# MaxHalford/sorobn

Hardware: NVIDIA H100
Metric: exact-inference queries/sec (higher is better)
Workload: dtype f32

## Files before the change

sorobn_b200/csrc/sbn_api.cu:

```cuda
#include <cuda_runtime.h>

#include <algorithm>
#include <cmath>
#include <cstdarg>
#include <cstdio>
#include <cstdlib>
#include <cstring>
#include <string>
#include <vector>

#include "sbn_chain.h"
#include "sbn_count.cuh"
#include "sbn_deriv.cuh"
#include "sbn_gibbs.cuh"
#include "sbn_internal.h"
#include "sbn_join.h"
#include "sbn_kernels.cuh"
#include "sbn_launch.h"
#include "sbn_marginal.cuh"
#include "sbn_mpe.cuh"
#include "sbn_pair.h"
#include "sbn_sample.cuh"
#include "sbn_soft.cuh"
#include "sbn_tma.h"
// ... 1095 lines not shown
        sbn_soft_pack<float><<<grid, threads, 0, stream>>>(static_cast<const float *>(P->lik), P->ld_lik, rows, n_soft,
                                                           P->d_soft, P->d_arena, P->ld, P->d_log_max);
    return cudaGetLastError();
}

inline bool hoisted(const sbn_program *P, const StepDesc &st) { return P->mode == 1 && st.kind == 0; }

inline bool chain_on(const sbn_program *P) {
    return P->use_chain && P->chain_fits && P->use_tiled && !P->use_branches && !P->segments.empty();
}

inline bool pair_on(const sbn_program *P) {
    return P->use_pair && P->use_tiled && !P->use_branches && (!chain_on(P) || P->pairs_avoid_segments) && !P->pairs.empty();
}

int run_table_steps(sbn_program *P) {
    if (P->mode != 1) return SBN_OK;
    SbnStep q;
    for (const StepDesc &st : P->steps) {
        if (!hoisted(P, st)) continue;
        build_params(P, st, nullptr, 0, 1, &q);
        SBN_CUDA(launch_step(P, st, q, P->stream));
    }
    SBN_CUDA(cudaStreamSynchronize(P->stream));
    P->setup_launches = P->launches;
    P->launches = 0;
    return SBN_OK;
}

inline bool fold_normalise(const sbn_program *P, const StepDesc &st, const SbnStep &q) {
#if !SBN_FOLD_NORMALISE
    (void)P;
    (void)st;
    (void)q;
    return false;
#endif
    static const bool enabled = [] {
        const char *e = getenv("SOROBN_B200_FOLD_NORMALISE");
        return e ? atoi(e) != 0 : true;
    }();
    return enabled && P->kind == kPosterior && !P->f64 && P->post_batched && st.kind == 1 && q.tile_off != nullptr &&
           q.slab_off == nullptr && st.n_tiles == 1 && st.n_out == P->Q && !sbn_tma_eligible(P, st);
}

int issue_all(sbn_program *P, const uint8_t *d_ev, int64_t ld_ev, int64_t n_rows, float *d_out, int64_t ld_out,
              cudaStream_t stream, cudaEvent_t *events, const DrawnCodes &dc = {}) {
    if (P->kind == kSample) SBN_CUDA(cudaMemsetAsync(dc.flags(P), 0, static_cast<size_t>(n_rows), stream));
    if (!P->soft.empty()) SBN_CUDA(launch_soft_pack(P, n_rows, stream));
    SbnStep q;
    int k = 0;
    int n_decoded = 0;
    bool folded = false;
    bool skip_second = false;
    for (const StepDesc &st : P->steps) {
        if (events) SBN_CUDA(cudaEventRecord(events[k], stream));
        ++k;
        if (hoisted(P, st)) continue;
        if (P->forward_run && !P->forward[k - 1]) continue;
        if (st.kind >= 2) {
            const int decoded = st.kind == 4 || st.kind == 5 ? n_decoded++ : 0;
            SBN_CUDA(launch_kind_step(P, st, decoded, d_ev, ld_ev, n_rows, d_out, ld_out, dc, stream));
            continue;
        }
        const int seg = chain_on(P) ? P->seg_first[k - 1] : -1;
        if (seg == -2) continue;
        if (seg >= 0) {
            P->launches++;
            SBN_CUDA(sbn_chain_launch(P, *P->segments[seg], d_ev, ld_ev, n_rows, d_out, ld_out, stream));
            continue;
        }
        int pair = pair_on(P) ? P->pair_first[k - 1] : -1;
        if (pair == -2 && !skip_second) pair = -1;
        skip_second = false;
        if (pair == -2) continue;
        if (pair >= 0 && !sbn_pair_fits(P, *P->pairs[pair])) pair = -1;
        if (pair >= 0) {
            skip_second = true;
            P->launches++;
            SBN_CUDA(sbn_pair_launch(P, *P->pairs[pair], d_ev, ld_ev, n_rows, stream));
            continue;
        }
        build_params(P, st, d_ev, ld_ev, n_rows, &q);
        if (k == static_cast<int>(P->steps.size()) && fold_normalise(P, st, q)) {
            q.norm_out = d_out;
            q.norm_ld = ld_out;
            q.norm_totals = P->d_total;
            q.norm_min = SBN_MIN_TOTAL_F32;
            folded = true;
        }
        SBN_CUDA(launch_step(P, st, q, stream));
    }
    if (events) SBN_CUDA(cudaEventRecord(events[k], stream));
    switch (P->kind) {
        case kPosterior:
            if (!folded && !(chain_on(P) && P->segments.back()->ends_in_posterior))
                SBN_CUDA(launch_normalise(P, d_out, ld_out, n_rows, stream));
            break;
        case kCounts:
        case kGrad: SBN_CUDA(launch_prob(P, n_rows, d_out, nullptr, stream)); break;
        case kSample: SBN_CUDA(launch_prob(P, n_rows, d_out, dc.flags(P), stream)); break;
        case kMarginals:
        case kMpe:
        case kMap: break;
    }
    if (events) SBN_CUDA(cudaEventRecord(events[k + 1], stream));
    return SBN_OK;
}

int issue_branched(sbn_program *P, const uint8_t *d_ev, int64_t ld_ev, int64_t n_rows, float *d_out, int64_t ld_out,
                   cudaStream_t origin) {
    const int n_steps = static_cast<int>(P->steps.size());
    const int n_slots = static_cast<int>(P->slots.size());
    std::vector<int> last_writer(n_slots, -1);
    std::vector<std::vector<int>> readers(n_slots);
    std::vector<int> stream_of(n_steps, 0);
    cudaEvent_t fork = P->step_done[n_steps];
    if (!P->soft.empty()) SBN_CUDA(launch_soft_pack(P, n_rows, origin));
    SBN_CUDA(cudaEventRecord(fork, origin));
    bool joined[sbn_program::kBranches] = {false, false, false, false};
    int rr = 0;
    SbnStep q;
    for (int s = 0; s < n_steps; ++s) {
        const StepDesc &st = P->steps[s];
        if (hoisted(P, st)) continue;
        std::vector<int> deps;
        int home = -1;
        int64_t home_size = -1;
        for (const InDesc &in : st.in) {
// ... 227 lines not shown
    if (n_table_floats > 0) {
        SBN_CUDA_P(cudaMalloc(&P->d_tables, static_cast<size_t>(n_table_floats) * elem));
        SBN_CUDA_P(cudaMemcpyAsync(P->d_tables, tables, static_cast<size_t>(n_table_floats) * elem,
                                   cudaMemcpyHostToDevice, P->stream));
    }
    int64_t shared_floats = 0;
    for (Slot &s : P->slots)
        if (!s.batched) shared_floats += round_up(s.padded, 64);
    if (shared_floats > 0) {
        SBN_CUDA_P(cudaMalloc(&P->d_shared, static_cast<size_t>(shared_floats) * elem));
        SBN_CUDA_P(cudaMemsetAsync(P->d_shared, 0, static_cast<size_t>(shared_floats) * elem, P->stream));
        int64_t off = 0;
        for (Slot &s : P->slots)
            if (!s.batched) {
                s.ptr = reinterpret_cast<float *>(reinterpret_cast<char *>(P->d_shared) + off * elem);
                off += round_up(s.padded, 64);
            }
    }
    {
        std::vector<int32_t> &tile_words = P->h_tile_words;
        tile_words.clear();
        plan_tiles(P, &tile_words);
        if (!tile_words.empty()) {
            SBN_CUDA_P(cudaMalloc(&P->d_tile_off, tile_words.size() * 4));
            SBN_CUDA_P(cudaMemcpyAsync(P->d_tile_off, tile_words.data(), tile_words.size() * 4,
                                       cudaMemcpyHostToDevice, P->stream));
        }
        SBN_CUDA_P(cudaStreamSynchronize(P->stream));
        if (P->kind == kPosterior && P->soft.empty()) sbn_chain_plan(P);
    }
    if (!P->soft.empty()) {
        P->use_tma = false;
        std::vector<int32_t> desc;
        for (const auto &sv : P->soft) {
            int64_t off = 0;
            for (int s = 0; s < sv.first; ++s)
                if (P->slots[s].batched) off += P->slots[s].size;
            desc.push_back(static_cast<int32_t>(off));
            desc.push_back(sv.second);
        }
        SBN_CUDA_P(cudaMalloc(&P->d_soft, desc.size() * 4));
        SBN_CUDA_P(cudaMemcpyAsync(P->d_soft, desc.data(), desc.size() * 4, cudaMemcpyHostToDevice, P->stream));
        SBN_CUDA_P(cudaStreamSynchronize(P->stream));
    }
    {
        static bool done[64] = {false};
        if (device < 64 && !done[device]) {
            SBN_CUDA_P(sbn_batched_set_attrs());
            SBN_CUDA_P(set_tiled_attrs());
            SBN_CUDA_P(sbn_chain_set_attrs());
            SBN_CUDA_P(sbn_tma_set_attrs());
            SBN_CUDA_P(sbn_join_set_attrs());
            SBN_CUDA_P(sbn_triple_rows_set_attrs());
            SBN_CUDA_P(sbn_marginal_set_attrs());
            SBN_CUDA_P(sbn_count_set_attrs());
            SBN_CUDA_P(sbn_deriv_set_attrs());
            SBN_CUDA_P(sbn_sample_set_attrs());
            SBN_CUDA_P(sbn_argmax_set_attrs());
            SBN_CUDA_P(sbn_batched_logdomain_set_attrs());
            done[device] = true;
        }
    }
    if (P->kind == kCounts || P->kind == kGrad) {
        for (const StepDesc &st : P->steps)
            if (st.kind == 3)
                P->partial_doubles = std::max<int64_t>(P->partial_doubles, count_grid(P, st, INT32_MAX) * SBN_COUNT_WARPS * st.span);
        SBN_CUDA_P(cudaMalloc(&P->d_counts, static_cast<size_t>(P->n_counts) * 8));
    }
#undef SBN_CUDA_P
    rc = run_table_steps(P);
    if (rc != SBN_OK) return bail(rc);
    {
        cudaError_t e = P->kind == kPosterior ? sbn_pair_plan(P) : cudaSuccess;
        if (e != cudaSuccess) return bail(fail(SBN_E_CUDA, "planning the paired steps failed: %s", cudaGetErrorString(e)));
    }
    *out = P;
    return SBN_OK;
}

int sbn_program_create(int device, const int32_t *words, int64_t n_words, const float *tables, int64_t n_table_floats,
                       sbn_program **out) {
    return create_common(device, words, n_words, tables, n_table_floats, false, out);
}

int sbn_program_create_f64(int device, const int32_t *words, int64_t n_words, const double *tables,
                           int64_t n_table_doubles, sbn_program **out) {
    return create_common(device, words, n_words, tables, n_table_doubles, true, out);
}

void sbn_program_destroy(sbn_program *P) {
    if (!P) return;
    cudaSetDevice(P->device);
    free_scratch(P);
    sbn_chain_free(P);
    sbn_pair_free(P);
    cudaFree(P->d_shared);
    cudaFree(P->d_counts);
    cudaFree(P->d_partial);
    cudaFree(P->d_drawn);
    cudaFree(P->d_sample_args);
    cudaFree(P->d_soft);
    cudaFree(P->d_tile_off);
    cudaFree(P->d_tables);
    if (P->stream) cudaStreamDestroy(P->stream);
    for (auto &b : P->branch)
        if (b) cudaStreamDestroy(b);
// ... 621 lines not shown
int sbn_program_mpe_soft_host(sbn_program *P, const uint8_t *ev, int64_t ld_ev, int64_t n_rows, const double *lik,
                              int64_t ld_lik, int lik_on_device, uint8_t *codes, double *log_prob) {
    if (!log_prob) return fail(SBN_E_INVALID, "null output");
    std::vector<float> lp(n_rows > 0 ? static_cast<size_t>(n_rows) : 0);
    std::vector<double> log_max(lp.size());
    const SoftLik soft = {true, lik, ld_lik, lik_on_device, log_max.data()};
    const int rc = sample_host_common(P, ev, ld_ev, n_rows, 1, 0, 0, codes, lp.data(), false, kMpe, soft);
    if (rc != SBN_OK) return rc;
    for (size_t i = 0; i < lp.size(); ++i) log_prob[i] = static_cast<double>(lp[i]) + log_max[i];
    return SBN_OK;
}

int sbn_program_profile(sbn_program *P, const uint8_t *d_ev, int64_t ld_ev, int64_t n_rows, float *d_out,
                        int64_t ld_out, void *stream_, float *step_ms, int64_t n_step_ms) {
    int rc = check_run_args(P, d_ev, ld_ev, n_rows, d_out, ld_out);
    if (rc != SBN_OK) return rc;
    if (P->f64) return fail(SBN_E_INVALID, "profiling is for float32 programs");
    const int64_t n = static_cast<int64_t>(P->steps.size()) + 1;
    if (!step_ms || n_step_ms < n) return fail(SBN_E_INVALID, "step_ms needs %lld entries", (long long)n);
    rc = reserve_rows(P, n_rows);
    if (rc != SBN_OK) return rc;
    if (n_rows > P->reserved_rows) return fail(SBN_E_NOMEM, "n_rows exceeds the scratch that fits the device");
    cudaStream_t stream = static_cast<cudaStream_t>(stream_);
    std::vector<cudaEvent_t> ev(n + 1);
    for (auto &e : ev) SBN_CUDA(cudaEventCreate(&e));
    rc = issue_all(P, d_ev, ld_ev, n_rows, d_out, ld_out, stream, ev.data());
    if (rc == SBN_OK) {
        cudaError_t e = cudaStreamSynchronize(stream);
        if (e != cudaSuccess) rc = fail(SBN_E_CUDA, "profile run failed: %s", cudaGetErrorString(e));
    }
    if (rc == SBN_OK)
        for (int64_t i = 0; i < n; ++i) cudaEventElapsedTime(&step_ms[i], ev[i], ev[i + 1]);
    for (auto &e : ev) cudaEventDestroy(e);
    return rc;
}

int sbn_program_info(const sbn_program *P, int64_t *info, int64_t n_info) {
    if (!P || !info || n_info < 8) return fail(SBN_E_INVALID, "info needs at least 8 entries");
    if (n_info >= 12) {
        int64_t covered = 0, hbm = 0, scratch = 0;
        for (const SbnSegment *seg : P->segments) {
            covered += static_cast<int64_t>(seg->steps.size());
            hbm += seg->hbm_bytes_per_row;
            scratch = std::max(scratch, seg->scratch_floats);
        }
        info[8] = chain_on(P) ? static_cast<int64_t>(P->segments.size()) : 0;
        info[9] = chain_on(P) ? covered : 0;
        info[10] = chain_on(P) ? hbm : 0;
        info[11] = scratch;
    }
    if (n_info >= 14) {
        int64_t saved = 0;
        for (const SbnPair *pr : P->pairs) saved += 8 * P->steps[pr->step1].n_out;
        info[12] = pair_on(P) ? static_cast<int64_t>(P->pairs.size()) : 0;
        info[13] = pair_on(P) ? saved : 0;
    }
    info[0] = P->Q;
    info[1] = P->n_ev;
    info[2] = static_cast<int64_t>(P->steps.size());
    info[3] = batched_floats_per_row(P);
    info[4] = P->reserved_rows;
    info[5] = P->launches;
    info[6] = P->mode;
    int64_t shared = 0;
    for (const Slot &s : P->slots)
        if (!s.batched) shared += s.size;
    info[7] = shared;
    return SBN_OK;
}

int sbn_program_step_roles(const sbn_program *P, int32_t *roles, int64_t n_roles) {
    if (!P || !roles || n_roles < static_cast<int64_t>(P->steps.size())) return fail(SBN_E_INVALID, "roles needs n_steps entries");
    int first_kind = 0;
    bool second_follows = false;
    for (size_t i = 0; i < P->steps.size(); ++i) {
        const StepDesc &st = P->steps[i];
        if (P->mode != 1 || hoisted(P, st)) {
            roles[i] = 0;
            continue;
        }
        roles[i] = 1;
        if (chain_on(P) && P->seg_first[i] != -1) {
            roles[i] = 6;
            continue;
        }
        int pair = pair_on(P) ? P->pair_first[i] : -1;
        if (pair == -2 && !second_follows) pair = -1;
        second_follows = false;
        if (pair == -2) roles[i] = first_kind == 1 ? 5 : 3;
        if (pair >= 0 && sbn_pair_fits(P, *P->pairs[pair])) {
            first_kind = P->pairs[pair]->kind;
            roles[i] = first_kind == 1 ? 4 : 2;
            second_follows = true;
        }
    }
    return SBN_OK;
}

int sbn_program_set_graph(sbn_program *P, int enabled) {
    if (!P) return fail(SBN_E_INVALID, "null program");
    P->use_graph = enabled != 0;
    P->use_branches = enabled == 3;
    drop_graphs(P);
    return SBN_OK;
}

// ... 395 lines not shown
```

sorobn_b200/csrc/sbn_internal.h:

```cpp
#pragma once
#include <cuda_runtime.h>
#include <stdint.h>

#include <string>
#include <utility>
#include <vector>

#include "../../include/sorobn_b200.h"

struct EvAxis {
    int col, stride, card;
};
struct InDesc {
    bool is_slot;
    int id;
    bool batched;
    int sx;
    std::vector<EvAxis> ev;
    std::vector<int> estrides;
    std::vector<int> strides;
};
struct StepDesc {
    int kind;
    int out_slot;
    int cx;
    int64_t n_out;
    std::vector<int> cards;
    std::vector<int> ecards;
    int64_t zoff_pos = -1;
    int64_t zoff_tiled_pos = -1;
    std::vector<InDesc> in;
    int tile = 0;
    int nu = 0, na = 0, nb = 0, nc = 0;
    std::vector<int> order;
    int64_t n_tiles = 0;
    int64_t tile_off_pos = 0;
    bool slab = false;
    bool big_tables = false;
    int slab_ma = 0, n_slab = 0;
    int64_t slab_off_pos = 0;
    int64_t slab_tile_off_pos = 0;
    int64_t tiles_per_super = 0, n_super = 0;
    int64_t slice_pos = -1;
    int64_t slice_tpc = 0;
    int64_t slice_smem = 0;
    int64_t q_offset = -1;
    int n_common = 0;
    std::vector<EvAxis> key;
    std::vector<int> cstrides;
    int64_t span = 0;
    int64_t soff_pos = -1, coff_pos = -1;
    bool logsumexp = false;
};
struct Slot {
    bool batched;
    int64_t size;
    int64_t padded;
    float *ptr;
};

inline int64_t round_up(int64_t v, int64_t m) { return (v + m - 1) / m * m; }

struct SbnSegment;
struct SbnPair;

enum ProgramKind {
    kPosterior,
    kMarginals,
    kCounts,
    kSample,
    kMpe,
    kMap,
    kGrad,
};

inline bool sbn_log_domain(ProgramKind k) { return k == kMpe || k == kMap; }

struct GraphKey {
    const void *ev = nullptr;
    int64_t ld_ev = 0, n_rows = 0;
    const void *out = nullptr;
    int64_t ld_out = 0;
    const void *partial = nullptr;
    const void *drawn = nullptr;
    int64_t n_draws = 0, ld_drawn = 0;
    const void *lik = nullptr;
    int64_t ld_lik = 0;
    const void *weight = nullptr;
    bool operator==(const GraphKey &o) const {
        return ev == o.ev && out == o.out && ld_ev == o.ld_ev && n_rows == o.n_rows && ld_out == o.ld_out &&
               partial == o.partial && drawn == o.drawn && n_draws == o.n_draws && ld_drawn == o.ld_drawn &&
               lik == o.lik && ld_lik == o.ld_lik && weight == o.weight;
    }
};
struct CachedGraph {
    cudaGraphExec_t exec = nullptr;
    GraphKey key;
    int64_t launches = 0;
};

struct sbn_program {
    int device = 0;
    int n_sms = 1;
    bool f64 = false;
    ProgramKind kind = kPosterior;
    int mode = 0, n_ev = 0, Q = 0, post_slot = 0, post_batched = 0;
    int64_t n_counts = 0;
    int64_t n_table_floats = 0;
    double *d_counts = nullptr;
    double *d_partial = nullptr;
    int64_t partial_doubles = 0;
    int n_sampled = 0;
    uint8_t *d_drawn = nullptr;
    int64_t drawn_bytes = 0;
    uint32_t *d_sample_args = nullptr;
    std::vector<std::pair<int, int>> soft;
    int n_lik = 0;
// ... 2 lines not shown
    double *d_log_max = nullptr;
    const void *lik = nullptr;
    int64_t ld_lik = 0;
    std::vector<char> forward;
    double *d_weight = nullptr;
    const double *weight = nullptr;
    bool forward_run = false;
    CachedGraph forward_graph;
    std::vector<std::pair<int64_t, int64_t>> tables;
    std::vector<int64_t> table_padded;
    float *d_tables = nullptr;
    std::vector<Slot> slots;
    std::vector<StepDesc> steps;

    int64_t reserved_rows = 0;
    int64_t ld = 0;
    float *d_arena = nullptr;
    float *d_shared = nullptr;
    int32_t *d_tile_off = nullptr;
    float *d_total = nullptr;
    uint8_t *d_ev = nullptr;
    float *d_out = nullptr;
    cudaStream_t stream = nullptr;
    static constexpr int kBranches = 4;
    cudaStream_t branch[kBranches] = {nullptr, nullptr, nullptr, nullptr};
    std::vector<cudaEvent_t> step_done;
    std::vector<cudaEvent_t> pipe_events;
    bool use_branches = false;

    bool use_graph = true;
    bool use_tiled = true;
    bool use_slab = true;
    bool use_preload = true;
    CachedGraph graph;
    CachedGraph pipe_graph;

    int64_t launches = 0;
    int64_t setup_launches = 0;

    std::vector<SbnSegment *> segments;
    std::vector<int> seg_first;
    float *d_chain_scratch = nullptr;
    bool use_chain = true;
    bool use_tma = true;
    bool chain_fits = true;
    std::vector<int32_t> h_tile_words;

    std::vector<SbnPair *> pairs;
    std::vector<int> pair_first;
    float *d_pair_canon = nullptr;
    int32_t *d_pair_tiles = nullptr;
    bool use_pair = true;
    bool pairs_avoid_segments = false;
};
```

sorobn_b200/csrc/sbn_pair.cu:

```cuda
#include "sbn_pair.h"

#include <algorithm>
#include <cstdlib>
#include <cstring>

#include "sbn_internal.h"
#include "sbn_kernels.cuh"
#include "sbn_launch.h"

namespace {

constexpr int kV = 2;

__device__ __forceinline__ void pair_coef8(float (&c)[SBN_PAIR_PW], const float *s) {
    const float4 lo = *reinterpret_cast<const float4 *>(s);
    const float4 hi = *reinterpret_cast<const float4 *>(s + 4);
    c[0] = lo.x, c[1] = lo.y, c[2] = lo.z, c[3] = lo.w;
    c[4] = hi.x, c[5] = hi.y, c[6] = hi.z, c[7] = hi.w;
}

template <int V>
__device__ __forceinline__ void pair_ev_offsets(const SbnPairParams &p, const SbnPairEv &d, int b, int (&e)[V]) {
#pragma unroll
    for (int l = 0; l < V; ++l) e[l] = 0;
// ... 105 lines not shown
    PairG G;
    G.p = p.g + b;
    G.base = 0;
    if constexpr (M1 == SBN_PAIR_GB || M1 == SBN_PAIR_GC) {
#pragma unroll
        for (int d = 0; d < T; ++d) {
            G.x[d] = static_cast<uint32_t>(d * p.g_x) * ld;
            G.d0[d] = static_cast<uint32_t>(d * p.g_y) * ld;
            G.d1[d] = static_cast<uint32_t>(d * p.g_w) * ld;
        }
    }
    const int t_begin = chunk * p.tiles_per_cta;
    const int t_end = min(p.n_tiles, t_begin + p.tiles_per_cta);

    for (int t = t_begin; t < t_end; ++t) {
        const int4 r0 = __ldg(reinterpret_cast<const int4 *>(p.tile_off) + 2 * t);
        const int4 r1 = __ldg(reinterpret_cast<const int4 *>(p.tile_off) + 2 * t + 1);
        const uint32_t ob = static_cast<uint32_t>(r0.x) * ld, fb = static_cast<uint32_t>(r0.y) * ld;

        float f[T][T][V];
#pragma unroll
        for (int x = 0; x < T; ++x)
#pragma unroll
            for (int y = 0; y < T; ++y) sbn_ldv<V>(f[x][y], fp + (fb + xs[x] + ys[y]));
        if (p.has_pre1) {
            const float *const k = s_canon + r1.x;
#pragma unroll
            for (int x = 0; x < T; ++x)
#pragma unroll
                for (int y = 0; y < T; ++y)
#pragma unroll
                    for (int l = 0; l < V; ++l) f[x][y][l] *= k[g1[l] + x * T + y];
        }
        float mid[T][T][V];
        if constexpr (M1 == SBN_PAIR_GB || M1 == SBN_PAIR_GC) G.base = static_cast<uint32_t>(r1.z) * ld;
        pair_step<M1, V>(f, mid, s_canon + r0.z, e1, G);
        if (p.has_pre2) {
            const float *const k = s_canon + r1.y;
#pragma unroll
            for (int y = 0; y < T; ++y)
#pragma unroll
                for (int w = 0; w < T; ++w)
#pragma unroll
                    for (int l = 0; l < V; ++l) mid[y][w][l] *= k[g2[l] + y * T + w];
        }
        float acc[T][T][V];
        pair_step<M2, V>(mid, acc, s_canon + r0.w, e2, G);

#pragma unroll
        for (int z = 0; z < T; ++z)
#pragma unroll
            for (int w = 0; w < T; ++w)
                if (w < p.cw && z < p.cz) sbn_stv<V>(op + (ob + ow[w] + oz[z]), acc[w][z]);
    }
}

template <int MINB>
__global__ void __launch_bounds__(SBN_TRIPLE_THREADS, MINB) sbn_triple_kernel(const __grid_constant__ SbnTripleParams p) {
    constexpr int T = SBN_PAIR_T;
    sbn_pdl_entry();
    const int rblock = blockIdx.x / p.n_chunks;
    const int chunk = blockIdx.x % p.n_chunks;
    const int b = rblock * static_cast<int>(blockDim.x) + threadIdx.x;
    if (b >= p.n_rows) return;
    const uint32_t ld = static_cast<uint32_t>(p.ld);
    const int g = threadIdx.y;
    const float *const ap = p.a + b + static_cast<uint32_t>(g * p.a_g) * ld;
    const float *const bp = p.b + b;
    const float *const cp = p.c + b;
    float *const op = p.out + b + static_cast<uint32_t>(g * p.o_g) * ld;
    uint32_t ak[T], aj[T], bj[T], bs[T], ck[T], cz[T];
#pragma unroll
    for (int d = 0; d < T; ++d) {
        ak[d] = static_cast<uint32_t>(d * p.a_k) * ld, aj[d] = static_cast<uint32_t>(d * p.a_j) * ld;
        bj[d] = static_cast<uint32_t>(d * p.b_j) * ld, bs[d] = static_cast<uint32_t>(d * p.b_s) * ld;
        ck[d] = static_cast<uint32_t>(d * p.c_k) * ld, cz[d] = static_cast<uint32_t>(d * p.c_z) * ld;
    }
    const uint32_t oz = static_cast<uint32_t>(p.o_z) * ld, os = static_cast<uint32_t>(p.o_s) * ld;
    const int t_begin = chunk * p.tiles_per_cta;
    const int t_end = min(p.n_tiles, t_begin + p.tiles_per_cta);
    for (int t = t_begin; t < t_end; ++t) {
        const int4 row = __ldg(reinterpret_cast<const int4 *>(p.tile_off) + t);
        float acc[T][T];
#pragma unroll
        for (int z = 0; z < T; ++z)
#pragma unroll
            for (int s = 0; s < T; ++s) acc[z][s] = 0.f;
#pragma unroll 1
        for (int pp = 0; pp < T; ++pp) {
            float A[T][T], B[T][T], C[T][T];
            const uint32_t a0 = static_cast<uint32_t>(row.y + pp * p.a_p) * ld, b0 = static_cast<uint32_t>(row.z + pp * p.b_p) * ld,
                           c0 = static_cast<uint32_t>(row.w + pp * p.c_p) * ld;
#pragma unroll
            for (int j = 0; j < T; ++j)
#pragma unroll
                for (int s = 0; s < T; ++s) B[j][s] = bp[b0 + bj[j] + bs[s]];
#pragma unroll
            for (int k = 0; k < T; ++k)
#pragma unroll
                for (int j = 0; j < T; ++j) A[k][j] = ap[a0 + ak[k] + aj[j]];
#pragma unroll
            for (int k = 0; k < T; ++k)
#pragma unroll
                for (int z = 0; z < T; ++z) C[k][z] = cp[c0 + ck[k] + cz[z]];
#pragma unroll
            for (int k = 0; k < T; ++k) {
// ... 250 lines not shown
            kg = k;
    int64_t n_tiles = 1;
    std::vector<int> r2;
    for (int k = 0; k < n2; ++k)
        if (k != ks && k != kz && k != kg) r2.push_back(k), n_tiles *= s2.cards[k];
    if (n_tiles >= (1LL << 27)) return nullptr;

    SbnPair *pr = new SbnPair();
    memset(&pr->q, 0, sizeof pr->q);
    memset(&pr->t, 0, sizeof pr->t);
    pr->kind = 1;
    pr->step1 = i1, pr->step2 = i2;
    pr->g_in = -1;
    pr->a_in = ai, pr->b_in = 1 - ai, pr->c_in = 1 - mi;
    pr->tile_off_pos = static_cast<int64_t>(tiles->size());
    SbnTripleParams &q = pr->t;
    q.n_tiles = static_cast<int32_t>(n_tiles);
    q.a_j = A.estrides[0], q.a_k = A.strides[jk], q.a_p = A.strides[jp];
    q.b_j = B.estrides[0], q.b_s = B.strides[to1[ks]], q.b_p = B.strides[jp];
    q.c_k = C.estrides[kk], q.c_p = C.estrides[1 - kk], q.c_z = C.strides[kz];
    int64_t os = 1;
    std::vector<int64_t> os2(n2);
    for (int k = 0; k < n2; ++k) os2[k] = os, os *= s2.cards[k];
    q.o_z = static_cast<int32_t>(os2[kz]);
    q.o_s = static_cast<int32_t>(os2[ks]);
    q.group = kg >= 0 ? T : 1;
    q.o_g = kg >= 0 ? static_cast<int32_t>(os2[kg]) : 0;
    q.a_g = kg >= 0 ? A.strides[to1[kg]] : 0;
    std::vector<int> dig(r2.size(), 0);
    for (int64_t t = 0; t < n_tiles; ++t) {
        int64_t ob = 0, ab = 0, bb = 0, cb = 0;
        for (size_t k = 0; k < r2.size(); ++k) {
            const int ax = r2[k];
            ob += dig[k] * os2[ax];
            cb += static_cast<int64_t>(dig[k]) * C.strides[ax];
            if (to1[ax] >= 0) {
                ab += static_cast<int64_t>(dig[k]) * A.strides[to1[ax]];
                bb += static_cast<int64_t>(dig[k]) * B.strides[to1[ax]];
            }
        }
        tiles->push_back(static_cast<int32_t>(ob));
        tiles->push_back(static_cast<int32_t>(ab));
        tiles->push_back(static_cast<int32_t>(bb));
        tiles->push_back(static_cast<int32_t>(cb));
        for (size_t k = 0; k < dig.size(); ++k) {
            if (++dig[k] < s2.cards[r2[k]]) break;
            dig[k] = 0;
        }
    }
    sbn_triple_rows_plan(q, tiles->data() + pr->tile_off_pos, &pr->rows);
    return pr;
}

}

cudaError_t sbn_pair_set_attrs() {
    return cudaSuccess;
}

void sbn_pair_free(sbn_program *P) {
    for (SbnPair *pr : P->pairs) delete pr;
    P->pairs.clear();
    P->pair_first.clear();
    cudaFree(P->d_pair_canon);
    cudaFree(P->d_pair_tiles);
    P->d_pair_canon = nullptr;
    P->d_pair_tiles = nullptr;
}

cudaError_t sbn_pair_plan(sbn_program *P) {
    constexpr int T = SBN_PAIR_T;
    P->pair_first.assign(P->steps.size(), -1);
    if (P->mode != 1 || P->f64) return cudaSuccess;
    static const int min_card = [] {
        const char *e = getenv("SOROBN_B200_PAIR_MIN_CARD");
        return e ? atoi(e) : 4;
    }();

    static const bool triples_on = [] {
        const char *e = getenv("SOROBN_B200_TRIPLE");
        return e ? atoi(e) != 0 : true;
    }();

    HostTables H;
    std::vector<float> canon;
    std::vector<int32_t> tiles;
    cudaError_t err = cudaSuccess;
    bool fetched = false;

    const int n_steps = static_cast<int>(P->steps.size());
    auto launched = [&](int i) { return P->steps[i].kind != 0; };
    P->pairs_avoid_segments = P->use_chain && !P->segments.empty();
    auto in_segment = [&](int i) { return P->pairs_avoid_segments && P->seg_first[i] != -1; };
    for (int i1 = 0; i1 < n_steps; ++i1) {
        if (!launched(i1) || P->pair_first[i1] != -1) continue;
        int i2 = i1 + 1;
        while (i2 < n_steps && !launched(i2)) ++i2;
        if (i2 >= n_steps) break;
        if (in_segment(i1) || in_segment(i2)) continue;
        const StepDesc &s1 = P->steps[i1], &s2 = P->steps[i2];
        if (triples_on) {
            if (SbnPair *tr = plan_triple(P, i1, i2, &tiles)) {
                P->pair_first[i1] = static_cast<int>(P->pairs.size());
                P->pair_first[i2] = -2;
                P->pairs.push_back(tr);
                continue;
            }
        }
        if (s1.kind != 1 || s2.kind != 1 || s1.ecards.size() != 1 || s2.ecards.size() != 1) continue;
        if (s1.tile == 0 || s2.tile == 0) continue;
        int fi = -1, gi = -1, mi = -1, n_b1 = 0, n_b2 = 0;
        for (int i = 0; i < static_cast<int>(s1.in.size()); ++i)
            if (s1.in[i].batched) gi = fi, fi = i, ++n_b1;
        for (int i = 0; i < static_cast<int>(s2.in.size()); ++i)
            if (s2.in[i].batched) mi = i, ++n_b2;
        if (n_b1 < 1 || n_b1 > 2 || n_b2 != 1) continue;
// ... 70 lines not shown
            q.canon_floats = static_cast<int32_t>(total);
            const int64_t at_c1 = 0, at_c2 = c1.floats(), at_g1 = at_c2 + c2.floats(), at_g2 = at_g1 + g1.floats();
            canon.resize(canon.size() + static_cast<size_t>(total), 0.f);
            fill_canon(c1, canon.data() + pr->canon_pos + at_c1);
            fill_canon(c2, canon.data() + pr->canon_pos + at_c2);
            fill_canon(g1, canon.data() + pr->canon_pos + at_g1);
            fill_canon(g2, canon.data() + pr->canon_pos + at_g2);
            q.n_tiles = static_cast<int32_t>(n_tiles);
            q.f_sx = F.estrides[0];
            q.f_sy = F.strides[jy];
            q.cx = cx, q.cy = cy, q.cw = s2.cards[kw], q.cz = s2.cards[kz];
            int64_t os = 1;
            std::vector<int64_t> os2(n2);
            for (int k = 0; k < n2; ++k) os2[k] = os, os *= s2.cards[k];
            q.o_sw = static_cast<int32_t>(os2[kw]);
            q.o_sz = static_cast<int32_t>(os2[kz]);
            if (gi >= 0) q.g_x = s1.in[gi].estrides[0], q.g_y = s1.in[gi].strides[jy], q.g_w = s1.in[gi].strides[jw];
            q.has_pre1 = g1.tabs.empty() ? 0 : 1;
            q.has_pre2 = g2.tabs.empty() ? 0 : 1;
            set_ev(&q.ev_main1, c1);
            set_ev(&q.ev_main2, c2);
            set_ev(&q.ev_pre1, g1);
            set_ev(&q.ev_pre2, g2);
            std::vector<int> dig(r2.size(), 0);
            for (int64_t t = 0; t < n_tiles; ++t) {
                int64_t ob = 0, fb = 0;
                for (size_t k = 0; k < r2.size(); ++k) {
                    ob += dig[k] * os2[r2[k]];
                    fb += static_cast<int64_t>(dig[k]) * F.strides[r1[k]];
                }
                tiles.push_back(static_cast<int32_t>(ob));
                tiles.push_back(static_cast<int32_t>(fb));
                tiles.push_back(static_cast<int32_t>(at_c1 + tile_slab(c1, r1, dig)));
                tiles.push_back(static_cast<int32_t>(at_c2 + tile_slab(c2, r2, dig)));
                tiles.push_back(static_cast<int32_t>(at_g1 + tile_slab(g1, r1, dig)));
                tiles.push_back(static_cast<int32_t>(at_g2 + tile_slab(g2, r2, dig)));
                int64_t gb = 0;
                if (gi >= 0)
                    for (size_t k = 0; k < r1.size(); ++k) gb += static_cast<int64_t>(dig[k]) * s1.in[gi].strides[r1[k]];
                tiles.push_back(static_cast<int32_t>(gb));
                tiles.push_back(0);
                for (size_t k = 0; k < dig.size(); ++k) {
                    if (++dig[k] < s2.cards[r2[k]]) break;
                    dig[k] = 0;
                }
            }
            P->pair_first[i1] = static_cast<int>(P->pairs.size());
            P->pair_first[i2] = -2;
            P->pairs.push_back(pr);
            break;
        }
    }
    if (P->pairs.empty()) return cudaSuccess;
    err = cudaMalloc(&P->d_pair_canon, std::max<size_t>(canon.size(), 4) * 4);
    if (err != cudaSuccess) return err;
    err = cudaMalloc(&P->d_pair_tiles, tiles.size() * 4);
    if (err != cudaSuccess) return err;
    if (!canon.empty()) err = cudaMemcpy(P->d_pair_canon, canon.data(), canon.size() * 4, cudaMemcpyHostToDevice);
    if (err != cudaSuccess) return err;
    return cudaMemcpy(P->d_pair_tiles, tiles.data(), tiles.size() * 4, cudaMemcpyHostToDevice);
}

static cudaError_t triple_launch(sbn_program *P, const SbnPair &pr, int64_t n_rows, cudaStream_t stream) {
    SbnTripleParams q = pr.t;
    const StepDesc &s1 = P->steps[pr.step1], &s2 = P->steps[pr.step2];
    q.a = P->slots[s1.in[pr.a_in].id].ptr;
    q.b = P->slots[s1.in[pr.b_in].id].ptr;
    q.c = P->slots[s2.in[pr.c_in].id].ptr;
    q.out = P->slots[s2.out_slot].ptr;
    q.ld = P->ld;
    q.n_rows = static_cast<int32_t>(n_rows);
    q.tile_off = P->d_pair_tiles + pr.tile_off_pos;
    if (sbn_triple_rows_launch(P, pr.rows, q, stream)) return cudaGetLastError();
    const int rows_per_cta = q.group > 1 ? 32 : 128;
    const int64_t n_rblocks = (n_rows + rows_per_cta - 1) / rows_per_cta;
    static const int64_t tpc_env = [] {
        const char *e = getenv("SOROBN_B200_TRIPLE_TPC");
        return e ? atoll(e) : 1LL;
    }();
    static const int minb = [] {
        const char *e = getenv("SOROBN_B200_TRIPLE_MINB");
        return e ? atoi(e) : 3;
    }();
    const int64_t tpc = std::max<int64_t>(1, std::min<int64_t>(q.n_tiles, tpc_env));
    q.tiles_per_cta = static_cast<int32_t>(tpc);
    q.n_chunks = static_cast<int32_t>((q.n_tiles + tpc - 1) / tpc);
    const int64_t grid = q.n_chunks * n_rblocks;
    if (grid >= (1LL << 31)) return cudaErrorInvalidConfiguration;
    const dim3 g(static_cast<unsigned>(grid)), b(rows_per_cta, q.group);
    if (minb == 3) sbn_launch(sbn_triple_kernel<3>, g, b, 0, stream, q);
    else if (minb == 1) sbn_launch(sbn_triple_kernel<1>, g, b, 0, stream, q);
    else sbn_launch(sbn_triple_kernel<2>, g, b, 0, stream, q);
    return cudaGetLastError();
}

bool sbn_pair_fits(const sbn_program *P, const SbnPair &pr) {
    const StepDesc &s1 = P->steps[pr.step1], &s2 = P->steps[pr.step2];
    int64_t entries = P->slots[s2.out_slot].size;
    for (const InDesc &in : s1.in)
        if (in.batched) entries = std::max(entries, P->slots[in.id].size);
    for (const InDesc &in : s2.in)
        if (in.batched && in.id != s1.out_slot) entries = std::max(entries, P->slots[in.id].size);
    const char *e = getenv("SOROBN_B200_PAIR_IDX_LIMIT");
    const int64_t limit = e ? atoll(e) : (1LL << 31);
    return entries * P->ld < limit;
}

cudaError_t sbn_pair_launch(sbn_program *P, const SbnPair &pr, const uint8_t *d_ev, int64_t ld_ev, int64_t n_rows,
                            cudaStream_t stream) {
    if (pr.kind == 1) return triple_launch(P, pr, n_rows, stream);
    SbnPairParams q = pr.q;
    const StepDesc &s1 = P->steps[pr.step1], &s2 = P->steps[pr.step2];
    q.f = P->slots[s1.in[pr.f_in].id].ptr;
    q.g = pr.g_in >= 0 ? P->slots[s1.in[pr.g_in].id].ptr : q.f;
    q.out = P->slots[s2.out_slot].ptr;
    q.ev = d_ev;
    q.ld_ev = ld_ev;
    q.ld = P->ld;
    q.n_rows = static_cast<int32_t>(n_rows);
    q.canon = P->d_pair_canon + pr.canon_pos;
    q.tile_off = P->d_pair_tiles + pr.tile_off_pos;
    const int64_t n_rblocks = (n_rows + SBN_PAIR_ROWS - 1) / SBN_PAIR_ROWS;
    static const int64_t target_env = [] {
        const char *e = getenv("SOROBN_B200_PAIR_CTAS");
        return e ? atoll(e) : 0LL;
    }();
    const int64_t target = target_env > 0 ? target_env : 8LL * P->n_sms * 6;
    const int64_t chunks = std::max<int64_t>(1, std::min<int64_t>(q.n_tiles, target / std::max<int64_t>(1, n_rblocks)));
    const int64_t tpc = (q.n_tiles + chunks - 1) / chunks;
    q.tiles_per_cta = static_cast<int32_t>(tpc);
    q.n_chunks = static_cast<int32_t>((q.n_tiles + tpc - 1) / tpc);
    const int64_t grid = q.n_chunks * n_rblocks;
    if (grid >= (1LL << 31)) return cudaErrorInvalidConfiguration;
    launch_modes(pr, q, static_cast<unsigned>(grid), static_cast<size_t>(q.canon_floats) * 4, stream);
    return cudaGetLastError();
}
```

sorobn_b200/csrc/sbn_pair.h:

```cpp
#pragma once
#include <cuda_runtime.h>
#include <stdint.h>

#include <vector>

#include "../../include/sorobn_b200.h"

#define SBN_PAIR_T 5
#define SBN_PAIR_PW 8
#define SBN_PAIR_MAX_EV 4
#define SBN_PAIR_ROWS 256
#define SBN_TRIPLE_THREADS 160
#define SBN_PAIR_SMEM_MAX (40 * 1024)

struct SbnPairEv {
    int32_t n;
    int32_t col[SBN_PAIR_MAX_EV], stride[SBN_PAIR_MAX_EV], card[SBN_PAIR_MAX_EV];
};

struct SbnPairParams {
    const float *f;
    float *out;
    const uint8_t *ev;
    const float *canon;
// ... 3 lines not shown
    int32_t canon_floats;
    int32_t n_tiles, tiles_per_cta, n_chunks;
    int32_t f_sx, f_sy;
    int32_t cx, cy, cw, cz;
    int32_t o_sw, o_sz;
    int32_t has_pre1, has_pre2;
    SbnPairEv ev_main1, ev_main2, ev_pre1, ev_pre2;
    const float *g;
    int32_t g_x, g_y, g_w;
};

enum SbnPairMode { SBN_PAIR_B = 0, SBN_PAIR_CU = 1, SBN_PAIR_CE = 2, SBN_PAIR_GB = 3, SBN_PAIR_GC = 4 };

struct SbnTripleParams {
    const float *a, *b, *c;
    float *out;
    const int32_t *tile_off;
    int64_t ld;
    int32_t n_rows;
    int32_t n_tiles, tiles_per_cta, n_chunks;
    int32_t a_p, a_k, a_j;
    int32_t b_p, b_j, b_s;
    int32_t c_p, c_k, c_z;
    int32_t o_z, o_s;
    int32_t group;
    int32_t a_g, o_g;
};

#define SBN_TRIPLE_ROWS_R 16
#define SBN_TRIPLE_ROWS_COMBOS 25
#define SBN_TRIPLE_ROWS_MIN_COMBOS 8
struct SbnTripleRows {
    int ok;
    int n_combos;
    int32_t u_card[3], u_stride[3];
    int32_t u_dig[3][SBN_TRIPLE_ROWS_COMBOS];
    int32_t o_off[SBN_TRIPLE_ROWS_COMBOS];
};

struct SbnPair {
    int kind;
    int step1, step2;
    int f_in;
    int g_in;
    int m1, m2;
    SbnPairParams q;
    SbnTripleParams t;
    SbnTripleRows rows;
    int a_in, b_in, c_in;
    int64_t tile_off_pos;
    int64_t canon_pos;
};

struct sbn_program;
cudaError_t sbn_pair_plan(sbn_program *P);
cudaError_t sbn_pair_launch(sbn_program *P, const SbnPair &pr, const uint8_t *d_ev, int64_t ld_ev, int64_t n_rows,
                            cudaStream_t stream);
bool sbn_pair_fits(const sbn_program *P, const SbnPair &pr);
cudaError_t sbn_pair_set_attrs();
void sbn_pair_free(sbn_program *P);

void sbn_triple_rows_plan(const SbnTripleParams &q, const int32_t *tiles, SbnTripleRows *rows);
bool sbn_triple_rows_launch(const sbn_program *P, const SbnTripleRows &rows, const SbnTripleParams &q, cudaStream_t stream);
cudaError_t sbn_triple_rows_set_attrs();
```

Before: 25.03 million.

## Fuse consecutive pair launches into one chain kernel with shared-memory intermediates

After: 26.42 million (median of 6 runs). 1.06x the previous value.

```diff
diff --git a/sorobn_b200/csrc/sbn_api.cu b/sorobn_b200/csrc/sbn_api.cu
--- a/sorobn_b200/csrc/sbn_api.cu
+++ b/sorobn_b200/csrc/sbn_api.cu
@@ -1171,11 +1171,13 @@
     int n_decoded = 0;
     bool folded = false;
     bool skip_second = false;
+    int chain_through = -1;
     for (const StepDesc &st : P->steps) {
         if (events) SBN_CUDA(cudaEventRecord(events[k], stream));
         ++k;
         if (hoisted(P, st)) continue;
         if (P->forward_run && !P->forward[k - 1]) continue;
+        if (k - 1 <= chain_through) continue;
         if (st.kind >= 2) {
             const int decoded = st.kind == 4 || st.kind == 5 ? n_decoded++ : 0;
             SBN_CUDA(launch_kind_step(P, st, decoded, d_ev, ld_ev, n_rows, d_out, ld_out, dc, stream));
@@ -1193,6 +1195,18 @@
         skip_second = false;
         if (pair == -2) continue;
         if (pair >= 0 && !sbn_pair_fits(P, *P->pairs[pair])) pair = -1;
+        if (pair >= 0 && P->chain_at[pair] >= 0) {
+            const SbnPairChain &ch = P->pair_chains[P->chain_at[pair]];
+            bool fits = true;
+            for (int j = 1; j < ch.n; ++j) fits = fits && sbn_pair_fits(P, *P->pairs[ch.first + j]);
+            cudaError_t err = cudaSuccess;
+            if (fits && sbn_pair_chain_launch(P, ch, d_ev, ld_ev, n_rows, stream, &err)) {
+                SBN_CUDA(err);
+                P->launches++;
+                chain_through = ch.last_step;
+                continue;
+            }
+        }
         if (pair >= 0) {
             skip_second = true;
             P->launches++;
@@ -1526,6 +1540,7 @@
             SBN_CUDA_P(sbn_tma_set_attrs());
             SBN_CUDA_P(sbn_join_set_attrs());
             SBN_CUDA_P(sbn_triple_rows_set_attrs());
+            SBN_CUDA_P(sbn_pair_set_attrs());
             SBN_CUDA_P(sbn_marginal_set_attrs());
             SBN_CUDA_P(sbn_count_set_attrs());
             SBN_CUDA_P(sbn_deriv_set_attrs());
@@ -2253,6 +2268,7 @@
     if (n_info >= 14) {
         int64_t saved = 0;
         for (const SbnPair *pr : P->pairs) saved += 8 * P->steps[pr->step1].n_out;
+        for (const SbnPairChain &ch : P->pair_chains) saved += ch.saved_per_row;
         info[12] = pair_on(P) ? static_cast<int64_t>(P->pairs.size()) : 0;
         info[13] = pair_on(P) ? saved : 0;
     }
diff --git a/sorobn_b200/csrc/sbn_internal.h b/sorobn_b200/csrc/sbn_internal.h
--- a/sorobn_b200/csrc/sbn_internal.h
+++ b/sorobn_b200/csrc/sbn_internal.h
@@ -7,6 +7,7 @@
 #include <vector>
 
 #include "../../include/sorobn_b200.h"
+#include "sbn_pair.h"
 
 struct EvAxis {
     int col, stride, card;
@@ -62,7 +63,6 @@
 inline int64_t round_up(int64_t v, int64_t m) { return (v + m - 1) / m * m; }
 
 struct SbnSegment;
-struct SbnPair;
 
 enum ProgramKind {
     kPosterior,
@@ -171,4 +171,6 @@
     int32_t *d_pair_tiles = nullptr;
     bool use_pair = true;
     bool pairs_avoid_segments = false;
+    std::vector<SbnPairChain> pair_chains;
+    std::vector<int> chain_at;
 };
diff --git a/sorobn_b200/csrc/sbn_pair.cu b/sorobn_b200/csrc/sbn_pair.cu
--- a/sorobn_b200/csrc/sbn_pair.cu
+++ b/sorobn_b200/csrc/sbn_pair.cu
@@ -181,6 +181,172 @@
 #pragma unroll
             for (int w = 0; w < T; ++w)
                 if (w < p.cw && z < p.cz) sbn_stv<V>(op + (ob + ow[w] + oz[z]), acc[w][z]);
+    }
+}
+
+template <int V>
+__device__ __forceinline__ void pair_step_m(int mode, const float (&in)[SBN_PAIR_T][SBN_PAIR_T][V],
+                                            float (&acc)[SBN_PAIR_T][SBN_PAIR_T][V], const float *k, const int (&e)[V],
+                                            const PairG &G) {
+    switch (mode) {
+        case SBN_PAIR_B: pair_step<SBN_PAIR_B, V>(in, acc, k, e, G); break;
+        case SBN_PAIR_CU: pair_step<SBN_PAIR_CU, V>(in, acc, k, e, G); break;
+        case SBN_PAIR_CE: pair_step<SBN_PAIR_CE, V>(in, acc, k, e, G); break;
+        case SBN_PAIR_GB: pair_step<SBN_PAIR_GB, V>(in, acc, k, e, G); break;
+        default: pair_step<SBN_PAIR_GC, V>(in, acc, k, e, G); break;
+    }
+}
+
+struct SbnPairChainParams {
+    SbnPairParams q[SBN_PAIR_CHAIN_MAX];
+    int32_t m1[SBN_PAIR_CHAIN_MAX], m2[SBN_PAIR_CHAIN_MAX];
+    int32_t n_pairs;
+    int32_t canon_floats;
+    int32_t front_floats;
+    int32_t tiles;
+};
+
+constexpr int kChainR = SBN_PAIR_CHAIN_R;
+constexpr int kChainThreads = SBN_PAIR_CHAIN_TILES * SBN_PAIR_CHAIN_R / kV;
+
+__device__ __forceinline__ void chain_stage_canon(float *dst, const SbnPairParams &q) {
+    for (int i = threadIdx.x; i < q.canon_floats / 4; i += blockDim.x)
+        asm volatile("cp.async.cg.shared.global [%0], [%1], 16;" ::"r"(sbn_smem_u32(dst + 4 * i)), "l"(q.canon + 4 * i)
+                     : "memory");
+    asm volatile("cp.async.commit_group;" ::: "memory");
+}
+__device__ __forceinline__ void chain_canon_wait() { asm volatile("cp.async.wait_all;" ::: "memory"); }
+
+__global__ void __launch_bounds__(kChainThreads, SBN_PAIR_CHAIN_MINB) sbn_pair_chain_kernel(const __grid_constant__ SbnPairChainParams p) {
+    constexpr int T = SBN_PAIR_T, V = kV, R = kChainR, RT = R / V;
+    extern __shared__ __align__(16) float s_mem[];
+    float *const s_canon = s_mem;
+    float *const s_front = s_mem + p.canon_floats;
+    int *const s_evo = reinterpret_cast<int *>(s_front + p.front_floats);
+    int4 *const s_tiles = reinterpret_cast<int4 *>(s_evo + SBN_PAIR_CHAIN_MAX * 4 * R);
+    sbn_pdl_launch_dependents();
+
+    const int rg = threadIdx.x % RT, t = threadIdx.x / RT;
+    const int b = blockIdx.x * R + rg * V;
+    const bool live = b < p.q[0].n_rows;
+    float *const fs = s_front + rg * V;
+    chain_stage_canon(s_canon, p.q[0]);
+    for (int i = threadIdx.x; i < p.n_pairs * 4 * RT; i += blockDim.x) {
+        const int j = i / (4 * RT), a = i / RT % 4, g = i % RT;
+        const SbnPairParams &q = p.q[j];
+        const SbnPairEv &d = a == 0 ? q.ev_main1 : a == 1 ? q.ev_main2 : a == 2 ? q.ev_pre1 : q.ev_pre2;
+        const int bb = blockIdx.x * R + g * V;
+        int e[V];
+        pair_ev_offsets<V>(q, d, bb, e);
+#pragma unroll
+        for (int l = 0; l < V; ++l) s_evo[(j * 4 + a) * R + g * V + l] = e[l];
+    }
+    for (int i = threadIdx.x; i < p.n_pairs * p.tiles * 2; i += blockDim.x) {
+        const int j = i / (p.tiles * 2), k = i % (p.tiles * 2);
+        if (k < 2 * p.q[j].n_tiles) s_tiles[i] = __ldg(reinterpret_cast<const int4 *>(p.q[j].tile_off) + k);
+    }
+    chain_canon_wait();
+    __syncthreads();
+    sbn_pdl_wait();
+
+    for (int j = 0; j < p.n_pairs; ++j) {
+        const SbnPairParams &q = p.q[j];
+        const bool mine = live && t < q.n_tiles;
+        const bool last = j + 1 == p.n_pairs;
+        const uint32_t ld = static_cast<uint32_t>(q.ld);
+        float acc[T][T][V];
+        int4 r0 = make_int4(0, 0, 0, 0);
+        if (mine) {
+            int e1[V], e2[V], g1[V], g2[V];
+            const int *const ev = s_evo + j * 4 * R + rg * V;
+#pragma unroll
+            for (int l = 0; l < V; ++l) e1[l] = ev[l], e2[l] = ev[R + l], g1[l] = ev[2 * R + l], g2[l] = ev[3 * R + l];
+            r0 = s_tiles[(j * p.tiles + t) * 2];
+            const int4 r1 = s_tiles[(j * p.tiles + t) * 2 + 1];
+            float f[T][T][V];
+            if (j == 0) {
+                const float *const fp = q.f + b;
+                const uint32_t fb = static_cast<uint32_t>(r0.y) * ld;
+                uint32_t xs[T], ys[T];
+#pragma unroll
+                for (int d = 0; d < T; ++d) {
+                    xs[d] = static_cast<uint32_t>(min(d, q.cx - 1) * q.f_sx) * ld;
+                    ys[d] = static_cast<uint32_t>(min(d, q.cy - 1) * q.f_sy) * ld;
+                }
+#pragma unroll
+                for (int x = 0; x < T; ++x)
+#pragma unroll
+                    for (int y = 0; y < T; ++y) sbn_ldv<V>(f[x][y], fp + (fb + xs[x] + ys[y]));
+            } else {
+#pragma unroll
+                for (int x = 0; x < T; ++x)
+#pragma unroll
+                    for (int y = 0; y < T; ++y) {
+                        const int e = r0.y + min(x, q.cx - 1) * q.f_sx + min(y, q.cy - 1) * q.f_sy;
+                        const float2 v = *reinterpret_cast<const float2 *>(fs + e * R);
+                        f[x][y][0] = v.x, f[x][y][1] = v.y;
+                    }
+            }
+            if (q.has_pre1) {
+                const float *const k = s_canon + r1.x;
+#pragma unroll
+                for (int x = 0; x < T; ++x)
+#pragma unroll
+                    for (int y = 0; y < T; ++y)
+#pragma unroll
+                        for (int l = 0; l < V; ++l) f[x][y][l] *= k[g1[l] + x * T + y];
+            }
+            PairG G;
+            G.p = q.g + b;
+            G.base = 0;
+            if (p.m1[j] >= SBN_PAIR_GB) {
+                G.base = static_cast<uint32_t>(r1.z) * ld;
+#pragma unroll
+                for (int d = 0; d < T; ++d) {
+                    G.x[d] = static_cast<uint32_t>(d * q.g_x) * ld;
+                    G.d0[d] = static_cast<uint32_t>(d * q.g_y) * ld;
+                    G.d1[d] = static_cast<uint32_t>(d * q.g_w) * ld;
+                }
+            }
+            float mid[T][T][V];
+            pair_step_m<V>(p.m1[j], f, mid, s_canon + r0.z, e1, G);
+            if (q.has_pre2) {
+                const float *const k = s_canon + r1.y;
+#pragma unroll
+                for (int y = 0; y < T; ++y)
+#pragma unroll
+                    for (int w = 0; w < T; ++w)
+#pragma unroll
+                        for (int l = 0; l < V; ++l) mid[y][w][l] *= k[g2[l] + y * T + w];
+            }
+            pair_step_m<V>(p.m2[j], mid, acc, s_canon + r0.w, e2, G);
+        }
+        __syncthreads();
+        if (!last) chain_stage_canon(s_canon, p.q[j + 1]);
+        if (mine) {
+            if (last) {
+                float *const op = q.out + b;
+                const uint32_t ob = static_cast<uint32_t>(r0.x) * ld;
+#pragma unroll
+                for (int z = 0; z < T; ++z)
+#pragma unroll
+                    for (int w = 0; w < T; ++w)
+                        if (w < q.cw && z < q.cz)
+                            sbn_stv<V>(op + (ob + static_cast<uint32_t>(w * q.o_sw) * ld + static_cast<uint32_t>(z * q.o_sz) * ld),
+                                       acc[w][z]);
+            } else {
+#pragma unroll
+                for (int z = 0; z < T; ++z)
+#pragma unroll
+                    for (int w = 0; w < T; ++w)
+                        if (w < q.cw && z < q.cz)
+                            *reinterpret_cast<float2 *>(fs + (r0.x + w * q.o_sw + z * q.o_sz) * R) = make_float2(acc[w][z][0], acc[w][z][1]);
+            }
+        }
+        if (!last) {
+            chain_canon_wait();
+            __syncthreads();
+        }
     }
 }
 
@@ -537,16 +703,94 @@
     return pr;
 }
 
+size_t chain_smem_bytes(const SbnPairChain &ch) {
+    return static_cast<size_t>(ch.canon_floats + ch.front_entries * kChainR + SBN_PAIR_CHAIN_MAX * 4 * kChainR +
+                               static_cast<int64_t>(ch.n) * ch.tiles * 8) * 4;
+}
+
+void plan_chains(sbn_program *P) {
+    const int n_steps = static_cast<int>(P->steps.size());
+    const int n_pairs = static_cast<int>(P->pairs.size());
+    P->chain_at.assign(P->pairs.size(), -1);
+    auto next_launched = [&](int i) {
+        for (++i; i < n_steps; ++i)
+            if (P->steps[i].kind != 0) return i;
+        return n_steps;
+    };
+    auto sole_reader = [&](int slot, int writer, int reader) {
+        for (int i = writer + 1; i < n_steps; ++i) {
+            const StepDesc &st = P->steps[i];
+            for (const InDesc &in : st.in)
+                if (in.is_slot && in.id == slot && i != reader) return false;
+            if (st.out_slot == slot) return true;
+        }
+        return true;
+    };
+    auto follows = [&](const SbnPair &a, const SbnPair &b) {
+        if (a.kind != 0 || b.kind != 0 || next_launched(a.step2) != b.step1) return false;
+        const int mid = P->steps[a.step2].out_slot;
+        const StepDesc &s1 = P->steps[b.step1];
+        if (!s1.in[b.f_in].is_slot || s1.in[b.f_in].id != mid || mid == P->post_slot) return false;
+        if (b.g_in >= 0 && s1.in[b.g_in].id == mid) return false;
+        return sole_reader(mid, a.step2, b.step1);
+    };
+    static const int min_pairs = [] {
+        const char *e = getenv("SOROBN_B200_PAIR_CHAIN_MIN");
+        return std::max(2, e ? atoi(e) : SBN_PAIR_CHAIN_MIN);
+    }();
+    auto tiles_ok = [&](const SbnPair &pr) { return pr.kind == 0 && pr.q.n_tiles <= SBN_PAIR_CHAIN_TILES; };
+    for (int a = 0; a < n_pairs;) {
+        int e = a + 1;
+        while (e < n_pairs && e - a < SBN_PAIR_CHAIN_MAX && tiles_ok(*P->pairs[e - 1]) && tiles_ok(*P->pairs[e]) &&
+               follows(*P->pairs[e - 1], *P->pairs[e]))
+            ++e;
+        if (e - a >= min_pairs) {
+            SbnPairChain ch{};
+            ch.first = a, ch.n = e - a;
+            ch.last_step = P->pairs[e - 1]->step2;
+            for (int j = a; j < e; ++j) {
+                const SbnPair &pr = *P->pairs[j];
+                ch.tiles = std::max(ch.tiles, static_cast<int>(pr.q.n_tiles));
+                ch.canon_floats = std::max<int64_t>(ch.canon_floats, pr.q.canon_floats);
+                if (j + 1 < e) {
+                    const int64_t n = P->steps[pr.step2].n_out;
+                    ch.front_entries = std::max(ch.front_entries, n);
+                    ch.saved_per_row += 8 * n;
+                }
+            }
+            const int64_t smem = chain_smem_bytes(ch);
+            int resident = 0;
+            cudaOccupancyMaxActiveBlocksPerMultiprocessor(&resident, sbn_pair_chain_kernel, ch.tiles * kChainR / kV,
+                                                          static_cast<size_t>(smem));
+            cudaGetLastError();
+            if (resident >= SBN_PAIR_CHAIN_MINB) {
+                P->chain_at[a] = static_cast<int>(P->pair_chains.size());
+                P->pair_chains.push_back(ch);
+            }
+        }
+        a = e;
+    }
+}
+
+bool chain_enabled() {
+    const char *e = getenv("SOROBN_B200_PAIR_CHAIN");
+    return e ? atoi(e) != 0 : true;
+}
+
 }
 
 cudaError_t sbn_pair_set_attrs() {
-    return cudaSuccess;
+    return cudaFuncSetAttribute(sbn_pair_chain_kernel, cudaFuncAttributeMaxDynamicSharedMemorySize,
+                                SBN_PAIR_SMEM_MAX + SBN_PAIR_CHAIN_TILES * SBN_PAIR_T * SBN_PAIR_T * kChainR * 4 +
+                                    SBN_PAIR_CHAIN_MAX * (4 * kChainR + SBN_PAIR_CHAIN_TILES * 8) * 4);
 }
 
 void sbn_pair_free(sbn_program *P) {
     for (SbnPair *pr : P->pairs) delete pr;
     P->pairs.clear();
     P->pair_first.clear();
+    P->pair_chains.clear();
+    P->chain_at.clear();
     cudaFree(P->d_pair_canon);
     cudaFree(P->d_pair_tiles);
     P->d_pair_canon = nullptr;
@@ -723,6 +967,7 @@
         }
     }
     if (P->pairs.empty()) return cudaSuccess;
+    plan_chains(P);
     err = cudaMalloc(&P->d_pair_canon, std::max<size_t>(canon.size(), 4) * 4);
     if (err != cudaSuccess) return err;
     err = cudaMalloc(&P->d_pair_tiles, tiles.size() * 4);
@@ -806,3 +1051,37 @@
     launch_modes(pr, q, static_cast<unsigned>(grid), static_cast<size_t>(q.canon_floats) * 4, stream);
     return cudaGetLastError();
 }
+
+bool sbn_pair_chain_launch(sbn_program *P, const SbnPairChain &ch, const uint8_t *d_ev, int64_t ld_ev, int64_t n_rows,
+                           cudaStream_t stream, cudaError_t *err) {
+    if (!chain_enabled()) return false;
+    const int64_t n_blocks = (n_rows + kChainR - 1) / kChainR;
+    if (n_blocks < 2LL * SBN_PAIR_CHAIN_MINB * P->n_sms) return false;
+    SbnPairChainParams c;
+    memset(&c, 0, sizeof c);
+    c.n_pairs = ch.n;
+    c.canon_floats = static_cast<int32_t>(ch.canon_floats);
+    for (int j = 0; j < ch.n; ++j) {
+        const SbnPair &pr = *P->pairs[ch.first + j];
+        SbnPairParams &q = c.q[j];
+        q = pr.q;
+        const StepDesc &s1 = P->steps[pr.step1], &s2 = P->steps[pr.step2];
+        q.f = P->slots[s1.in[pr.f_in].id].ptr;
+        q.g = pr.g_in >= 0 ? P->slots[s1.in[pr.g_in].id].ptr : q.f;
+        q.out = P->slots[s2.out_slot].ptr;
+        q.ev = d_ev;
+        q.ld_ev = ld_ev;
+        q.ld = P->ld;
+        q.n_rows = static_cast<int32_t>(n_rows);
+        q.canon = P->d_pair_canon + pr.canon_pos;
+        q.tile_off = P->d_pair_tiles + pr.tile_off_pos;
+        c.m1[j] = pr.m1, c.m2[j] = pr.m2;
+    }
+    c.front_floats = static_cast<int32_t>(ch.front_entries * kChainR);
+    c.tiles = ch.tiles;
+    const size_t smem = chain_smem_bytes(ch);
+    sbn_launch(sbn_pair_chain_kernel, dim3(static_cast<unsigned>(n_blocks)), dim3(static_cast<unsigned>(ch.tiles * kChainR / kV)),
+               smem, stream, c);
+    *err = cudaGetLastError();
+    return true;
+}
diff --git a/sorobn_b200/csrc/sbn_pair.h b/sorobn_b200/csrc/sbn_pair.h
--- a/sorobn_b200/csrc/sbn_pair.h
+++ b/sorobn_b200/csrc/sbn_pair.h
@@ -79,11 +79,27 @@
     int64_t canon_pos;
 };
 
+#define SBN_PAIR_CHAIN_MAX 4
+#define SBN_PAIR_CHAIN_MIN 2
+#define SBN_PAIR_CHAIN_R 16
+#define SBN_PAIR_CHAIN_TILES 25
+#define SBN_PAIR_CHAIN_MINB 2
+struct SbnPairChain {
+    int first, n;
+    int last_step;
+    int tiles;
+    int64_t canon_floats;
+    int64_t front_entries;
+    int64_t saved_per_row;
+};
+
 struct sbn_program;
 cudaError_t sbn_pair_plan(sbn_program *P);
 cudaError_t sbn_pair_launch(sbn_program *P, const SbnPair &pr, const uint8_t *d_ev, int64_t ld_ev, int64_t n_rows,
                             cudaStream_t stream);
 bool sbn_pair_fits(const sbn_program *P, const SbnPair &pr);
+bool sbn_pair_chain_launch(sbn_program *P, const SbnPairChain &ch, const uint8_t *d_ev, int64_t ld_ev, int64_t n_rows,
+                           cudaStream_t stream, cudaError_t *err);
 cudaError_t sbn_pair_set_attrs();
 void sbn_pair_free(sbn_program *P);
 
```
